# chao1224/GeoSSL

Measured on AMD Instinct MI355X. Metric: molecules/s/GPU SchNet+DDM fwd+bwd (QM9-sized, bs=1024); % HBM roofline, higher is better.
Workload: dtype f32

## Files before the change

geossl_amd/csrc/aggregate_reg.h:

```cpp
#pragma once
#include "common.h"

namespace geossl {

typedef float f32x2 __attribute__((ext_vector_type(2)));

template <int NMAX, int RING_ = 0>
__device__ __forceinline__ void aggregate_reg_body(const float* __restrict__ x, const float* __restrict__ Wf,
                                                   const uint8_t* __restrict__ pair_flag, int a0, int n, int base,
                                                   int lane, int f, int F, int swap, float* __restrict__ out) {
#pragma clang fp contract(off)
  typedef f32x2 V;
#ifndef AGG_RING_SMALL
#define AGG_RING_SMALL 16
#endif
  constexpr int RING = RING_ > 0 ? RING_ : (NMAX > 26 ? 24 : (NMAX > 20 ? 20 : (NMAX > 18 ? 12 : AGG_RING_SMALL)));
  constexpr int NPOS = NMAX * (NMAX - 1) / 2;
  const float* __restrict__ wbase = Wf + (size_t)base * F;
  const bool has_cols = f >= 0;
  f = has_cols ? f : 0;
  if (n < 2) {
    if (n == 1 && has_cols) *reinterpret_cast<V*>(out + (size_t)a0 * F + f) = V(0.0f);
    return;
  }
  V xr[NMAX], acc[NMAX], ring[RING];
#pragma unroll
  for (int i = 0; i < NMAX; ++i) {
    xr[i] = *reinterpret_cast<const V*>(x + (size_t)(a0 + min(i, n - 1)) * F + f);
    acc[i] = V(0.0f);
  }
  const int nu = __builtin_amdgcn_readfirstlane(n);
  int rs_req = 0;
  auto load_row = [&](int a, int b) {
    asm volatile("" : "+s"(rs_req));
    const int slot = b < nu ? rs_req + (b - a - 1) : 0;
    const float* rowp = wbase + (size_t)slot * F;
    return __builtin_nontemporal_load(reinterpret_cast<const V*>(rowp + f));
  };
  auto next_pos = [&](int& a, int& b) {
    if (++b == NMAX) {
      rs_req += nu - a - 1;
      ++a;
      b = a + 1;
    }
  };
  unsigned flr[NMAX - 1];
#pragma unroll
  for (int a = 0; a < NMAX - 1; ++a) {
    const bool mine = lane > a && lane < n;
    flr[a] = pair_flag[base + (mine ? a * n - a * (a + 1) / 2 + lane - a - 1 : 0)];
  }
  int q = 0, ap = 0, bp = 1;
#pragma unroll
  for (int k = 0; k < RING && k < NPOS; ++k) {
    ring[k] = load_row(ap, bp);
    next_pos(ap, bp);
  }
#pragma unroll
  for (int a = 0; a < NMAX - 1; ++a) {
    const bool mine = lane > a && lane < n;
    unsigned fl = flr[a];
    asm volatile("" : "+v"(fl));
    fl = mine ? fl : 0u;
    if (swap) fl = ((fl & 1u) << 1) | ((fl >> 1) & 1u);
    const unsigned long long m0 = __builtin_amdgcn_ballot_w64((fl & 1u) != 0u);
    const unsigned long long m1 = __builtin_amdgcn_ballot_w64((fl & 2u) != 0u);
    V acc_a = acc[a];
    const V xa = xr[a];
#pragma unroll
    for (int b = a + 1; b < NMAX; ++b, ++q) {
      const V w = ring[q % RING];
      if (q + RING < NPOS) {
        ring[q % RING] = load_row(ap, bp);
        next_pos(ap, bp);
      }
      const V t0 = xr[b] * w;
      const V s0 = acc_a + t0;
      acc_a = ((m0 >> b) & 1ull) ? s0 : acc_a;
      const V t1 = xa * w;
      const V s1 = acc[b] + t1;
      acc[b] = ((m1 >> b) & 1ull) ? s1 : acc[b];
      asm volatile("" : "+v"(acc_a.x), "+v"(acc_a.y), "+v"(acc[b].x), "+v"(acc[b].y) : : "memory");
      __builtin_amdgcn_sched_barrier(0);
    }
    acc[a] = acc_a;
  }
#pragma unroll
  for (int i = 0; i < NMAX; ++i)
    if (i < n && has_cols) *reinterpret_cast<V*>(out + (size_t)(a0 + i) * F + f) = acc[i];
}

template <int NW = 4>
__device__ __forceinline__ void aggregate_block_body(const float* __restrict__ x, const float* __restrict__ Wf,
                                                     const uint8_t* __restrict__ pair_flag, int a0, int n, int base,
                                                     int swap, float* __restrict__ out, uint8_t* smem) {
#pragma clang fp contract(off)
  typedef f32x2 V;
  constexpr int F = 128, NP = 32;
  float* xs = reinterpret_cast<float*>(smem);
  uint8_t* fls = smem + 33 * F * sizeof(float);
  const int tid = threadIdx.x, lane = tid & 63;
  const int wave = __builtin_amdgcn_readfirstlane(tid >> 6);
  const int nu = __builtin_amdgcn_readfirstlane(n), np = nu * (nu - 1) / 2;
  for (int i = tid; i < nu * (F / 4); i += 64 * NW) {
    const int row = i >> 5, q = i & 31;
    *reinterpret_cast<f32x4*>(xs + row * F + 4 * q) = *reinterpret_cast<const f32x4*>(x + (size_t)(a0 + row) * F + 4 * q);
  }
  for (int p = tid; p < np; p += 64 * NW) {
    unsigned fl = pair_flag[base + p];
    if (swap) fl = ((fl & 1u) << 1) | ((fl >> 1) & 1u);
    fls[p] = (uint8_t)fl;
  }
  __syncthreads();
  if (nu < 2) {
    if (nu == 1 && wave == 0) *reinterpret_cast<V*>(out + (size_t)a0 * F + 2 * lane) = V(0.0f);
    return;
  }
  const float* __restrict__ wcol = Wf + (size_t)base * F + 2 * lane;
  const float* xl = xs + 2 * lane;
  int slot_l = 0, b_l = 0;
  unsigned long long mask = 0ull;
  auto describe = [&](int a) {
// ... 216 lines not shown
```

geossl_amd/csrc/chain.hip:

```cpp
#include "common.h"
#include "geossl_hip.h"
#include "split.h"
#ifdef LOOP_TIMING
__device__ long long loop_dbg[2 * 1024];
__device__ int loop_dbg_n;
#define LOOP_MARK(tag)                                                                                     \
  do {                                                                                                     \
    if (blockIdx.x == 5 && threadIdx.x == 64) {                                                            \
      const int k_ = loop_dbg_n;                                                                           \
      if (k_ < 1024) {                                                                                     \
        loop_dbg[2 * k_] = (tag);                                                                          \
        loop_dbg[2 * k_ + 1] = (long long)__builtin_amdgcn_s_memrealtime();                                \
        loop_dbg_n = k_ + 1;                                                                               \
      }                                                                                                    \
    }                                                                                                      \
  } while (0)
#else
#define LOOP_MARK(tag) do {} while (0)
#endif
#include "aggregate_reg.h"

#include <cstdlib>

using namespace geossl;
// ... 462 lines not shown
                  const u32x4* src = xs + (size_t)((ks + 1) * 3) * 64;
                  xn.h = src[0]; xn.m = src[64]; xn.l = src[128];
                }
                __builtin_amdgcn_sched_barrier(0);
                mma6(acc, af[ks], xa);
                __builtin_amdgcn_sched_barrier(0);
                if (ks + 1 < KS) xa = xn;
              }
            }
            epilogue(st, m, acc, tp, rs, v);
            if (s + 1 < NS) {
              const float lo[8] = {v[0], v[1], v[2], v[3], v[4], v[5], v[6], v[7]};
              const float hi[8] = {v[8], v[9], v[10], v[11], v[12], v[13], v[14], v[15]};
              const Frag3 f0 = split8(lo), f1 = split8(hi);
              u32x4* xd = xchg + (size_t)(s & 1) * CHUNK + (size_t)(2 * m * 3) * 64 + lane;
              xd[0] = f0.h; xd[64] = f0.m; xd[128] = f0.l;
              xd[192] = f1.h; xd[256] = f1.m; xd[320] = f1.l;
            }
          }
          __syncthreads();
          if (active && mbc == 0) store_v(st, m, ro, live, v);
          if (cc + NSLOT < total) issue(cc + NSLOT);
        }
      }
    }
  }
}

__device__ __forceinline__ float silu_f(float x) { return x / (1.0f + expf(-x)); }
__device__ __forceinline__ float dsilu_f(float x) {
  const float sg = 1.0f / (1.0f + expf(-x));
  return sg * (1.0f + x * (1.0f - sg));
}
template <int NS, int RB, int WPS, bool SILU, typename ChainT>
__device__ __forceinline__ void chain_cu_body(const ChainT& ch, const float* __restrict__ X, int ldx, int R,
                                              int row0, int row_end, int nloc) {
  constexpr int KS = 8, F = 128;
  constexpr int RBF = KS * 2 * 64;
#ifndef CHAIN_CU_NEB2
#define CHAIN_CU_NEB2 1
#endif
  constexpr int NEB = WPS == 1 ? 2 : CHAIN_CU_NEB2;
  extern __shared__ __attribute__((aligned(16))) uint8_t smem_raw[];
  u32x4* xbuf = reinterpret_cast<u32x4*>(smem_raw);
  float* bias_s = reinterpret_cast<float*>(xbuf + (size_t)RB * RBF);
  float* rmax = bias_s + NS * F;
  const int tid = threadIdx.x, lane = tid & 63, j = lane & 31, kh = lane >> 5;
  const int m = __builtin_amdgcn_readfirstlane(tid >> 6);
  const uint32_t voff = (uint32_t)lane * 16u;
  Frag2 af[KS];
  int eW = 0;
  float krow[RB];
  auto request_weights = [&](const auto& st) __attribute__((always_inline)) {
    const char* img = reinterpret_cast<const char*>(st.image) + (size_t)(m * KS) * 2 * 1024;
#pragma unroll
    for (int ks = 0; ks < KS; ++ks) {
      const char* bk = img + ks * 2 * 1024;
      asm volatile("" : "+s"(bk));
      af[ks].h = *reinterpret_cast<const u32x4*>(bk + voff);
      af[ks].l = *reinterpret_cast<const u32x4*>(bk + 1024 + voff);
    }
    eW = reinterpret_cast<const int*>(st.image)[4 * KS * 2 * 64 * 4 + m];
  };
  auto publish_max = [&](int i, float mx) __attribute__((always_inline)) {
    mx = fmaxf(mx, __shfl_xor(mx, 32, 64));
    if (kh == 0) rmax[(i * 4 + m) * 32 + j] = mx;
  };
  auto row_scale = [&](int i) __attribute__((always_inline)) {
    const float* r = rmax + (i * 4) * 32 + j;
    const float mx = fmaxf(fmaxf(r[0], r[32]), fmaxf(r[64], r[96]));
    const int e = mag_exponent(mx);
    krow[i] = __builtin_amdgcn_ldexpf(1.0f, e - 14);
    return __builtin_amdgcn_ldexpf(1.0f, 14 - e);
  };
  request_weights(ch.st[0]);
  for (int i = tid; i < NS * F; i += 256) {
    const int s = i / F;
    bias_s[i] = ch.st[s].bias != nullptr ? ch.st[s].bias[i - s * F] : 0.0f;
  }
  auto load_input = [&](const float* __restrict__ Xp, int ldxp) __attribute__((always_inline)) {
    f32x4 raw[RB][4];
    const char* xb = reinterpret_cast<const char*>(Xp) + 128 * m;
#pragma unroll
    for (int i = 0; i < RB; ++i) {
      const uint32_t rowc = (uint32_t)min(row0 + 32 * min(i, nloc - 1) + j, row_end - 1);
      const uint32_t xo = rowc * (uint32_t)ldxp * 4u + 16u * kh;
#pragma unroll
      for (int q = 0; q < 4; ++q) raw[i][q] = *reinterpret_cast<const f32x4*>(xb + 32 * q + xo);
    }
#pragma unroll
    for (int i = 0; i < RB; ++i) {
      if (i < nloc) {
        float mx = 0.0f;
#pragma unroll
        for (int q = 0; q < 4; ++q)
          mx = fmaxf(fmaxf(mx, fmaxf(fabsf(raw[i][q].x), fabsf(raw[i][q].y))), fmaxf(fabsf(raw[i][q].z), fabsf(raw[i][q].w)));
        publish_max(i, mx);
      }
    }
    lds_barrier();
#pragma unroll
    for (int i = 0; i < RB; ++i) {
      if (i < nloc) {
        const float sr = row_scale(i);
        const float lo[8] = {raw[i][0].x, raw[i][0].y, raw[i][0].z, raw[i][0].w,
                             raw[i][1].x, raw[i][1].y, raw[i][1].z, raw[i][1].w};
        const float hi[8] = {raw[i][2].x, raw[i][2].y, raw[i][2].z, raw[i][2].w,
                             raw[i][3].x, raw[i][3].y, raw[i][3].z, raw[i][3].w};
        const Frag2 f0 = split8h_scaled(lo, sr), f1 = split8h_scaled(hi, sr);
        u32x4* xd = xbuf + (size_t)i * RBF + (size_t)(2 * m * 2) * 64 + lane;
        xd[0] = f0.h; xd[64] = f0.l;
        xd[128] = f1.h; xd[192] = f1.l;
      }
    }
  };
  load_input(X, ldx);
  lds_barrier();
  LOOP_MARK(100);
  float vout[RB][16];
#pragma unroll
  for (int s = 0; s < NS; ++s) {
    const auto st = ch.st[s];
    const int eWs = eW;
    f32x4 tp[NEB][4], rs[NEB][4];
    const uint32_t nbytes = (uint32_t)R * (uint32_t)st.ld * 4u;
    const __amdgpu_buffer_rsrc_t rs_t = __builtin_amdgcn_make_buffer_rsrc(const_cast<float*>(st.tprev), 0, st.tprev != nullptr ? nbytes : 0u, 0x00020000);
    const __amdgpu_buffer_rsrc_t rs_r = __builtin_amdgcn_make_buffer_rsrc(const_cast<float*>(st.res), 0, st.res != nullptr ? nbytes : 0u, 0x00020000);
    const __amdgpu_buffer_rsrc_t rs_o = __builtin_amdgcn_make_buffer_rsrc(st.out, 0, st.out != nullptr ? nbytes : 0u, 0x00020000);
    const __amdgpu_buffer_rsrc_t rs_a = __builtin_amdgcn_make_buffer_rsrc(st.out_act, 0, (SILU && st.out_act != nullptr) ? nbytes : 0u, 0x00020000);
    const bool act_silu = SILU && (st.flags & GEOSSL_EPI_SILU) != 0;
    auto row_off = [&](int i) __attribute__((always_inline)) {
      const int row = row0 + 32 * i + j;
      return row < row_end ? (uint32_t)row * (uint32_t)st.ld * 4u + 128u * m + 16u * kh : 0xFFFFFF00u;
    };
    auto request_epi = [&](int i, f32x4 (&t)[4], f32x4 (&r)[4]) __attribute__((always_inline)) {
      const uint32_t ro = row_off(i);
#pragma unroll
      for (int q = 0; q < 4; ++q) t[q] = __builtin_bit_cast(f32x4, __builtin_amdgcn_raw_buffer_load_b128(rs_t, ro + 32 * q, 0, 0));
#pragma unroll
      for (int q = 0; q < 4; ++q) r[q] = __builtin_bit_cast(f32x4, __builtin_amdgcn_raw_buffer_load_b128(rs_r, ro + 32 * q, 0, 0));
    };
    auto store_rb = [&](int i) __attribute__((always_inline)) {
      const uint32_t ro = row_off(i);
#pragma unroll
      for (int q = 0; q < 4; ++q)
        __builtin_amdgcn_raw_buffer_store_b128(
            __builtin_bit_cast(u32x4, f32x4{vout[i][4 * q], vout[i][4 * q + 1], vout[i][4 * q + 2], vout[i][4 * q + 3]}), rs_o,
            ro + 32 * q, 0, 0);
      if constexpr (SILU) {
// ... 72 lines not shown
#pragma unroll
          for (int q = 0; q < 4; ++q) {
            vout[i][4 * q] *= dssp_from_out(t[q].x);
            vout[i][4 * q + 1] *= dssp_from_out(t[q].y);
            vout[i][4 * q + 2] *= dssp_from_out(t[q].z);
            vout[i][4 * q + 3] *= dssp_from_out(t[q].w);
          }
        }
        if (st.res != nullptr) {
#pragma unroll
          for (int q = 0; q < 4; ++q) {
            vout[i][4 * q] += r[q].x;
            vout[i][4 * q + 1] += r[q].y;
            vout[i][4 * q + 2] += r[q].z;
            vout[i][4 * q + 3] += r[q].w;
          }
        }
        if (s + 1 < NS) {
          float mx = 0.0f;
#pragma unroll
          for (int e = 0; e < 16; ++e) mx = fmaxf(mx, fabsf(vout[i][e]));
          publish_max(i, mx);
        }
        if (i > 0) store_rb(i - 1);
        if (i + 1 == nloc) store_rb(i);
      }
    }
    LOOP_MARK(110 + s);
    if (s + 1 < NS) {
      request_weights(ch.st[s + 1]);
      if (ch.st[s + 1].flags & GEOSSL_CHAIN_SAME_INPUT) continue;
      lds_barrier();
      if (ch.st[s + 1].flags & GEOSSL_CHAIN_NEW_INPUT) {
        load_input(ch.st[s + 1].xin, ch.st[s + 1].ldxin);
        lds_barrier();
        continue;
      }
#pragma unroll
      for (int i = 0; i < RB; ++i) {
        if (i < nloc) {
          const float sr = row_scale(i);
          float lo[8], hi[8];
#pragma unroll
          for (int e = 0; e < 8; ++e) {
            lo[e] = vout[i][e];
            hi[e] = vout[i][8 + e];
          }
          if constexpr (SILU) {
            if (st.flags & GEOSSL_EPI_SILU) {
#pragma unroll
              for (int e = 0; e < 8; ++e) {
                lo[e] = silu_f(lo[e]);
                hi[e] = silu_f(hi[e]);
              }
            }
          }
          const Frag2 f0 = split8h_scaled(lo, sr), f1 = split8h_scaled(hi, sr);
          u32x4* xd = xbuf + (size_t)i * RBF + (size_t)(2 * m * 2) * 64 + lane;
          xd[0] = f0.h; xd[64] = f0.l;
          xd[128] = f1.h; xd[192] = f1.l;
        }
      }
      lds_barrier();
    }
  }
}

template <int NS, int RB, int WPS, bool SILU>
__global__ __launch_bounds__(256, WPS) void k_row_chain_cu(GeosslChain ch, const float* __restrict__ X, int ldx, int R,
                                                           const int32_t* __restrict__ dyn_R) {
  R = dyn_count(R, dyn_R);
  const int nrb = (R + 31) / 32;
  const int nblk = (int)gridDim.x, base = nrb / nblk, extra = nrb - base * nblk, b = (int)blockIdx.x;
  const int rb0 = b * base + min(b, extra);
  const int nloc = base + (b < extra ? 1 : 0);
  if (nloc == 0) return;
  chain_cu_body<NS, RB, WPS, SILU>(ch, X, ldx, R, 32 * rb0, R, nloc);
}

struct LoopStage {
  const uint32_t* image;
  const float* bias;
  const float* res;
  const float* tprev;
  float* out;
  int flags, pad;
  static constexpr int ld = 128, ldxin = 0;
  static constexpr const float* xin = nullptr;
  static constexpr float* out_act = nullptr;
};
struct LoopOp {
  const float* X;
  const float* Wf;
  float* out;
  int kind, nstage, swap, pad;
  LoopStage st[3];
};
constexpr int LOOP_MAX_OPS = 14;
struct LoopArgs {
  LoopOp op[LOOP_MAX_OPS];
  const int4* plan;
  const int32_t* mol_ptr;
  const int32_t* pair_ptr;
  const uint8_t* pair_flag;
  int nops, R, stagger, pad;
  int nmol, mols_per_block;
};

template <int NMAX, int NW = 4>
__global__ __launch_bounds__(64 * NW, NW == 4 ? 2 : 1) void k_layer_loop(LoopArgs a) {
  constexpr int F = 128;
  int4 pl;
  if constexpr (NMAX > 0) {
    pl = a.plan[blockIdx.x];
  } else {
    pl.z = (int)blockIdx.x * a.mols_per_block;
    pl.w = min(pl.z + a.mols_per_block, a.nmol);
    if (pl.z >= pl.w) return;
    pl.x = a.mol_ptr[pl.z];
    pl.y = a.mol_ptr[pl.w];
    if (pl.x >= pl.y) return;
  }
  const int nloc = (pl.y - pl.x + 31) / 32;
  const int wave = __builtin_amdgcn_readfirstlane((int)threadIdx.x >> 6), lane = threadIdx.x & 63;
  if ((int)blockIdx.x >= ((int)gridDim.x + 1) / 2)
    for (int i = 0; i < a.stagger; ++i) __builtin_amdgcn_s_sleep(127);
  LOOP_MARK(1);
  for (int o = 0; o < a.nops; ++o) {
    const LoopOp& op = a.op[o];
    LOOP_MARK(10 + op.kind);
    if (op.kind == 0) {
      if (NW > 4 && wave >= 4) {
        for (int i = 0; i < 2 * op.nstage; ++i) __builtin_amdgcn_s_barrier();
      } else if (op.nstage == 1) chain_cu_body<1, 3, 2, false>(op, op.X, F, a.R, pl.x, pl.y, nloc);
      else if (op.nstage == 2) chain_cu_body<2, 3, 2, false>(op, op.X, F, a.R, pl.x, pl.y, nloc);
      else chain_cu_body<3, 3, 2, false>(op, op.X, F, a.R, pl.x, pl.y, nloc);
    } else {
      if constexpr (NMAX > 0 && NW == 4) {
        for (int mm = pl.z + wave; mm < pl.w; mm += 4) {
          const int a0 = a.mol_ptr[mm], n = a.mol_ptr[mm + 1] - a0, base = a.pair_ptr[mm];
          aggregate_reg_body<NMAX>(op.X, op.Wf, a.pair_flag, a0, n, base, lane, 2 * lane, F, op.swap, op.out);
        }
      } else {
        extern __shared__ __attribute__((aligned(16))) uint8_t loop_smem[];
        for (int mm = pl.z; mm < pl.w; ++mm) {
          const int a0 = a.mol_ptr[mm], n = a.mol_ptr[mm + 1] - a0, base = a.pair_ptr[mm];
          if (mm > pl.z) __syncthreads();
          aggregate_block_body<NW>(op.X, op.Wf, a.pair_flag, a0, n, base, op.swap, op.out, loop_smem);
        }
      }
    }
    LOOP_MARK(20);
    asm volatile("s_waitcnt vmcnt(0)" ::: "memory");
    LOOP_MARK(21);
    __syncthreads();
  }
  LOOP_MARK(2);
}

template <int KS>
int launch_chain(const GeosslChain& ch, const float* X, int ldx, int64_t R, hipStream_t stream,
                 const int32_t* dyn_R = nullptr) {
  constexpr int NMB = KS / 2, CHUNK_BYTES = KS * 3 * 1024;
  if (dyn_R != nullptr && KS != 8) return (int)hipErrorInvalidValue;
  const int nrb = (int)((R + 31) / 32), ngroups = (nrb + 3) / 4;
  const int nslot = chain_slots(ch.nstage * NMB);
  static const bool four_waves = getenv("GEOSSL_CHAIN4") != nullptr;
  static const bool eight_waves = getenv("GEOSSL_CHAIN8") != nullptr;
  const bool cu_form = KS == 8;
  const bool offsets32 = cu_form || !four_waves;
  bool same_input = false, silu = false;
  for (int s2 = 0; s2 < ch.nstage; ++s2) silu |= (ch.st[s2].flags & (GEOSSL_EPI_SILU | GEOSSL_EPI_MUL_DSILU)) != 0;
  if (ch.nstage > 3) silu = true;
  if (silu && !cu_form) return (int)hipErrorInvalidValue;
  for (int s2 = 0; s2 < ch.nstage; ++s2) {
    if (offsets32 && ((int64_t)R * ch.st[s2].ld * 4 >= (int64_t)0xFFFFFF00u || (int64_t)R * ldx * 4 >= (int64_t)0xFFFFFF00u ||
                      (int64_t)R * ch.st[s2].ldxin * 4 >= (int64_t)0xFFFFFF00u)) {
// ... 178 lines not shown
    } else if (src.kind == 1) {
      if (src.Wf == nullptr || src.out == nullptr) return (int)hipErrorInvalidValue;
      for (int s2 = 0; s2 < 3; ++s2) d.st[s2] = LoopStage{nullptr, nullptr, nullptr, nullptr, nullptr, 0, 0};
    } else {
      return (int)hipErrorInvalidValue;
    }
  }
  return 0;
}

static bool loop_wide(int64_t nblocks, bool one_molecule_per_block) {
  static int cus = 0;
  if (cus == 0) {
    int dev = 0, n = 0;
    cus = (hipGetDevice(&dev) == hipSuccess &&
           hipDeviceGetAttribute(&n, hipDeviceAttributeMultiprocessorCount, dev) == hipSuccess && n > 0) ? n : -1;
  }
  return one_molecule_per_block && cus > 0 && nblocks <= cus && getenv("GEOSSL_LOOP_NO_WIDE") == nullptr;
}

extern "C" int geossl_schnet_layer_loop(const GeosslLoopOp* ops, int nops, const int32_t* plan, int nblocks,
                                        const int32_t* mol_ptr, const int32_t* pair_ptr, const uint8_t* pair_flag,
                                        int max_n, int uniform, int64_t N, int F, int stagger, hipStream_t stream) {
  if (nops <= 0 || nblocks <= 0) return 0;
  if (ops == nullptr || plan == nullptr || nops > LOOP_MAX_OPS || F != 128 || !uniform || max_n > 20 || N <= 0)
    return (int)hipErrorInvalidValue;
  if (N * (int64_t)F * 4 >= (int64_t)0xFFFFFF00u) return (int)hipErrorInvalidValue;
  LoopArgs a;
  const int rc = fill_loop_ops(ops, nops, F, a);
  if (rc != 0) return rc;
  a.plan = reinterpret_cast<const int4*>(plan);
  a.mol_ptr = mol_ptr; a.pair_ptr = pair_ptr; a.pair_flag = pair_flag;
  a.nops = nops; a.R = (int)N; a.stagger = stagger; a.pad = 0; a.nmol = 0; a.mols_per_block = 0;
  const size_t lds = (size_t)3 * 8 * 2 * 1024 + (size_t)3 * 128 * sizeof(float) + (size_t)3 * 128 * sizeof(float);
  if (max_n <= 18) {
    allow_big_lds(&k_layer_loop<18>);
    hipLaunchKernelGGL((k_layer_loop<18>), dim3(nblocks), dim3(256), lds, stream, a);
  } else {
    allow_big_lds(&k_layer_loop<20>);
    hipLaunchKernelGGL((k_layer_loop<20>), dim3(nblocks), dim3(256), lds, stream, a);
  }
  GEOSSL_CHECK_LAUNCH();
  return 0;
}

extern "C" int geossl_schnet_layer_loop_ragged(const GeosslLoopOp* ops, int nops, const int32_t* mol_ptr,
                                               const int32_t* pair_ptr, const uint8_t* pair_flag, int64_t B,
                                               int mols_per_block, int64_t N, int F, hipStream_t stream) {
  if (nops <= 0 || B <= 0) return 0;
  if (ops == nullptr || mol_ptr == nullptr || pair_ptr == nullptr || nops > LOOP_MAX_OPS || F != 128 || N <= 0 ||
      mols_per_block < 1 || mols_per_block > 2)
    return (int)hipErrorInvalidValue;
  if (N * (int64_t)F * 4 >= (int64_t)0xFFFFFF00u) return (int)hipErrorInvalidValue;
  const int64_t nblocks = (B + mols_per_block - 1) / mols_per_block;
  if (nblocks > 1024) return (int)hipErrorInvalidValue;
  LoopArgs a;
  const int rc = fill_loop_ops(ops, nops, F, a);
  if (rc != 0) return rc;
  a.plan = nullptr;
  a.mol_ptr = mol_ptr; a.pair_ptr = pair_ptr; a.pair_flag = pair_flag;
  a.nops = nops; a.R = (int)N; a.stagger = 0; a.pad = 0; a.nmol = (int)B; a.mols_per_block = mols_per_block;
  const size_t lds = (size_t)3 * 8 * 2 * 1024 + (size_t)3 * 128 * sizeof(float) + (size_t)3 * 128 * sizeof(float);
  if (loop_wide(nblocks, mols_per_block == 1)) {
    allow_big_lds(&k_layer_loop<0, 8>);
    hipLaunchKernelGGL((k_layer_loop<0, 8>), dim3((unsigned)nblocks), dim3(512), lds, stream, a);
  } else {
// ... 7 lines not shown
```

geossl_amd/csrc/common.h:

```cpp
#pragma once
#include <hip/hip_runtime.h>
#include <stdint.h>

#include <mutex>

typedef float f32x16 __attribute__((ext_vector_type(16)));
typedef float f32x4 __attribute__((ext_vector_type(4)));

#define GEOSSL_MAX_LAYERS 12
#define GEOSSL_PI_F 3.14159265358979323846f

#define GEOSSL_CHECK_LAUNCH()                  \
  do {                                         \
    hipError_t e__ = hipGetLastError();        \
    if (e__ != hipSuccess) return (int)e__;    \
  } while (0)

namespace geossl {

inline void allow_big_lds_ptr(const void* kernel) {
  struct Seen { const void* fn; int dev; };
  static Seen seen[512];
  static int nseen = 0;
  static std::mutex mu;
// ... 75 lines not shown
    }
    asm volatile("s_waitcnt lgkmcnt(0)" ::: "memory");
#pragma unroll
    for (int u = 0; u < 2; ++u) {
      const int row16 = 8 * u + rr;
      const float4 v = *reinterpret_cast<const float4*>(stage + row16 * 32 + 4 * c4);
      consume(16 * half + row16, 4 * c4, v);
    }
    asm volatile("s_waitcnt lgkmcnt(0)" ::: "memory");
  }
}

__device__ __forceinline__ float pin(float v) {
  asm volatile("" : "+v"(v));
  return v;
}
__device__ __forceinline__ float4 pin(float4 v) {
  asm volatile("" : "+v"(v.x), "+v"(v.y), "+v"(v.z), "+v"(v.w));
  return v;
}

__device__ __forceinline__ float kahan_sum_strided(const float* __restrict__ p, int b0, int b1, int stride) {
#pragma clang fp reassociate(off) contract(off)
  float s = 0.0f, c = 0.0f;
#pragma unroll 4
  for (int b = b0; b < b1; ++b) {
    const float y = p[(size_t)b * stride] - c;
    const float t = s + y;
    c = (t - s) - y;
    s = t;
  }
  return s;
}

__device__ __forceinline__ int dyn_count(int cap, const int32_t* __restrict__ dyn) {
  return dyn != nullptr ? min(cap, *dyn) : cap;
}

__device__ __forceinline__ float wave_sum(float v) {
#pragma unroll
  for (int o = 32; o > 0; o >>= 1) v += __shfl_xor(v, o, 64);
  return v;
}

__device__ __forceinline__ float sigmoidf_(float v) { return 1.0f / (1.0f + expf(-v)); }
__device__ __forceinline__ float siluf_(float v) { return v / (1.0f + expf(-v)); }
__device__ __forceinline__ double softplus_d(double z) { return fmax(z, 0.0) + log1p(exp(-fabs(z))); }
__device__ __forceinline__ double sigmoid_d(double z) { return 1.0 / (1.0 + exp(-z)); }

enum Readout { kAdd = 0, kMean = 1, kExternal = 2 };

__device__ __forceinline__ float readout_col(const float* __restrict__ h, int F, int j, int a0, int a1, bool mean) {
  float acc = 0.0f;
  for (int a = a0; a < a1; ++a) acc += h[(size_t)a * F + j];
  return mean ? acc / fmaxf((float)(a1 - a0), 1.0f) : acc;
}
__device__ __forceinline__ float readout_grad(float g, int a0, int a1, bool mean) {
  return mean ? g / fmaxf((float)(a1 - a0), 1.0f) : g;
}
__device__ __forceinline__ void scatter_readout_col(float* __restrict__ dh, int F, int j, int a0, int a1, float g,
                                                    bool mean, bool accumulate = false) {
  const float gv = readout_grad(g, a0, a1, mean);
  for (int a = a0; a < a1; ++a) {
    const size_t o = (size_t)a * F + j;
    dh[o] = accumulate ? dh[o] + gv : gv;
  }
// ... 4 lines not shown
```

geossl_amd/csrc/ddm.hip:

```cpp
#include "common.h"
#include "geossl_hip.h"
#include "tn.h"
#include "wgrad.h"

using namespace geossl;

namespace {

inline int grid1d(int64_t n, int block, int cap = 2048) {
  int64_t g = (n + block - 1) / block;
  return (int)(g < 1 ? 1 : (g > cap ? cap : g));
}

__global__ __launch_bounds__(256) void k_sum_partial(const float* __restrict__ x, int64_t n, float* __restrict__ partial) {
  __shared__ float red[256];
  const int64_t per = (n + gridDim.x - 1) / gridDim.x;
  const int64_t lo = blockIdx.x * per, hi = min(n, lo + per);
  float s = 0.0f;
  for (int64_t i = lo + threadIdx.x; i < hi; i += 256) s += x[i];
  red[threadIdx.x] = s;
  __syncthreads();
  for (int o = 128; o > 0; o >>= 1) {
    if (threadIdx.x < o) red[threadIdx.x] += red[threadIdx.x + o];
    __syncthreads();
// ... 195 lines not shown
  const int a = grp * 4 + (threadIdx.x >> 6), lane = threadIdx.x & 63;
  if (a >= N) return;
  const int64_t p0 = inc_ptr[a], p1 = inc_ptr[a + 1];
  float acc[4] = {0.0f, 0.0f, 0.0f, 0.0f};
  if (accumulate) {
#pragma unroll
    for (int v = 0; v < 4; ++v)
      if (lane + 64 * v < F) acc[v] = dh[(size_t)a * F + lane + 64 * v];
  }
  for (int64_t pb = p0; pb < p1; pb += 64) {
    const int cnt = (int)min((int64_t)64, p1 - pb);
    const int mine = lane < cnt ? inc_idx[pb + lane] : 0;
    for (int q0 = 0; q0 < cnt; q0 += 8) {
      float val[8][4];
#pragma unroll
      for (int u = 0; u < 8; ++u) {
        const int s = __shfl(mine, min(q0 + u, cnt - 1), 64);
#pragma unroll
        for (int v = 0; v < 4; ++v)
          if (lane + 64 * v < F) val[u][v] = dfeat[(size_t)s * F + lane + 64 * v];
      }
#pragma unroll
      for (int u = 0; u < 8; ++u)
        if (q0 + u < cnt) {
#pragma unroll
          for (int v = 0; v < 4; ++v)
            if (lane + 64 * v < F) acc[v] += val[u][v];
        }
    }
  }
#pragma unroll
  for (int v = 0; v < 4; ++v)
    if (lane + 64 * v < F) dh[(size_t)a * F + lane + 64 * v] = acc[v];
}

__global__ void k_adam(float* __restrict__ p, const float* __restrict__ g, float* __restrict__ m,
                       float* __restrict__ v, int64_t n, float step_size, float w1, float beta2, float w2, float eps,
                       float wd, float bc2_sqrt, float grad_scale) {
  for (int64_t i = (int64_t)blockIdx.x * blockDim.x + threadIdx.x; i < n; i += (int64_t)gridDim.x * blockDim.x) {
    float gi = mul_rn(g[i], grad_scale);
    const float pi = p[i];
    if (wd != 0.0f) gi = fmaf(wd, pi, gi);
    const float m0 = m[i];
    const float mi = fmaf(w1, add_rn(gi, -m0), m0);
    const float vi = fmaf(w2, mul_rn(gi, gi), mul_rn(v[i], beta2));
    m[i] = mi;
    v[i] = vi;
    const float denom = add_rn(sqrtf(vi) / bc2_sqrt, eps);
    p[i] = fmaf(-step_size, mi / denom, pi);
  }
}

}

namespace geossl {
int launch_ncsn_small_reduce(const float* partial, int nblk, int F, const GeosslNcsnGrads& g, int accumulate,
                             hipStream_t stream);
}

extern "C" int64_t geossl_loss_reduce_workspace_floats(int64_t S) { return GEOSSL_LOSS_BLOCKS; }

extern "C" int geossl_loss_reduce(const float* loss_e, int64_t S, const int64_t* stats_divisor, float out_scale,
                                  float* loss, float* workspace, int accumulate, hipStream_t stream) {
  hipLaunchKernelGGL(k_sum_partial, dim3(GEOSSL_LOSS_BLOCKS), dim3(256), 0, stream, loss_e, S, workspace);
  GEOSSL_CHECK_LAUNCH();
  hipLaunchKernelGGL(k_loss_final, dim3(1), dim3(64), 0, stream, workspace, GEOSSL_LOSS_BLOCKS, stats_divisor, out_scale,
// ... 44 lines not shown
  int rc;
  o.dW[0] = grads->o2_w;
  o.db[0] = grads->o2_b;
  NcsnW2Ops l2{grow, w->o3_w, saved->a2, saved->a1, F, H};
  if (F == 128) rc = launch_wgrad_split<2, 4>(l2, 1, S, H, F, o, F, 1, workspace, accumulate, stream);
  else if (F == 64) rc = launch_wgrad_split<1, 2>(l2, 1, S, H, F, o, F, 1, workspace, accumulate, stream);
  else rc = launch_wgrad_split<1, 1>(l2, 1, S, H, F, o, F, 1, workspace, accumulate, stream);
  if (rc) return rc;
  o.dW[0] = grads->o1_w;
  o.db[0] = grads->o1_b;
  o.dd[0] = grads->o1_w + F;
  NcsnW1Ops l1{dz1, h, sei0, sei1, saved->emb, F};
  if (F == 128) rc = launch_wgrad_split<4, 4>(l1, 1, S, F, F, o, F + 1, F + 1, workspace, accumulate, stream);
  else if (F == 64) rc = launch_wgrad_split<2, 2>(l1, 1, S, F, F, o, F + 1, F + 1, workspace, accumulate, stream);
  else rc = launch_wgrad_split<1, 1>(l1, 1, S, F, F, o, F + 1, F + 1, workspace, accumulate, stream);
  if (rc) return rc;
  int chunk, nblk;
  small_plan(S, &chunk, &nblk);
  hipLaunchKernelGGL(k_ncsn_small_partial, dim3(nblk), dim3(128), 0, stream, *w, *saved, grow, demb, (int)S, F, chunk,
                     workspace);
  GEOSSL_CHECK_LAUNCH();
  return launch_ncsn_small_reduce(workspace, nblk, F, *grads, accumulate, stream);
}

namespace geossl {
int launch_ncsn_small_reduce(const float* partial, int nblk, int F, const GeosslNcsnGrads& g, int accumulate,
                             hipStream_t stream) {
  hipLaunchKernelGGL(k_ncsn_small_reduce, dim3(F / 2 + 3 * F + 2), dim3(64), 0, stream, partial, nblk, F, g, accumulate);
  GEOSSL_CHECK_LAUNCH();
  return 0;
}
}

extern "C" int geossl_incidence_gather(const float* dfeat, const int64_t* inc_ptr, const int32_t* inc_idx, int64_t N,
                                       int F, float* dh, int accumulate, hipStream_t stream) {
  if (N <= 0) return 0;
  const unsigned groups = (unsigned)((N + 3) / 4);
  hipLaunchKernelGGL(k_incidence_gather, dim3((groups + 7) / 8 * 8), dim3(256), 0, stream, dfeat, inc_ptr, inc_idx,
                     (int)N, F, dh, accumulate, (const float*)nullptr, (float*)nullptr, (const int32_t*)nullptr);
  GEOSSL_CHECK_LAUNCH();
  return 0;
}

namespace geossl {
int launch_incidence_gather2(const float* dfeat0, const float* dfeat1, const int64_t* inc_ptr, const int32_t* inc_idx,
                             int64_t N, int F, float* dh0, float* dh1, hipStream_t stream, const int32_t* dyn_view) {
  if (N <= 0) return 0;
  const unsigned groups = (unsigned)((N + 3) / 4);
  hipLaunchKernelGGL(k_incidence_gather, dim3((groups + 7) / 8 * 8, 2), dim3(256), 0, stream, dfeat0, inc_ptr, inc_idx,
                     (int)N, F, dh0, 0, dfeat1, dh1, dyn_view);
  GEOSSL_CHECK_LAUNCH();
  return 0;
}
}

extern "C" int geossl_adam_step(float* param, const float* grad, float* exp_avg, float* exp_avg_sq, int64_t n, double lr,
                                double beta1, double beta2, double eps, double weight_decay, int64_t step_count,
                                float grad_scale, hipStream_t stream) {
  if (n <= 0) return 0;
  const double bc1 = 1.0 - pow(beta1, (double)step_count);
  const double bc2 = 1.0 - pow(beta2, (double)step_count);
  hipLaunchKernelGGL(k_adam, dim3(grid1d(n, 256)), dim3(256), 0, stream, param, grad, exp_avg, exp_avg_sq, n,
                     (float)(lr / bc1), (float)(1.0 - beta1), (float)beta2, (float)(1.0 - beta2), (float)eps,
                     (float)weight_decay, (float)sqrt(bc2), grad_scale);
  GEOSSL_CHECK_LAUNCH();
  return 0;
}
```

geossl_amd/csrc/schnet.hip:

```cpp
#include "common.h"
#include "aggregate_reg.h"
#include "geossl_hip.h"
#include "tn.h"

#include <cstdlib>

using namespace geossl;

namespace {

inline int grid1d(int64_t n, int block, int cap = 2048) {
  int64_t g = (n + block - 1) / block;
  return (int)(g < 1 ? 1 : (g > cap ? cap : g));
}

__global__ void k_rbf(const float* __restrict__ d, int64_t E, const float* __restrict__ offset, int G, float coeff,
                      float* __restrict__ out) {
  for (int64_t i = (int64_t)blockIdx.x * blockDim.x + threadIdx.x; i < E * G; i += (int64_t)gridDim.x * blockDim.x) {
    const int64_t e = i / G;
    const int g = (int)(i - e * G);
    const float diff = d[e] - offset[g];
    out[i] = expf(coeff * (diff * diff));
  }
}
// ... 262 lines not shown
__global__ __launch_bounds__(256) void k_embedding_fwd4(const int64_t* __restrict__ z, int64_t zs,
                                                        const float* __restrict__ table, int C, int N,
                                                        float* __restrict__ out, int32_t* __restrict__ status,
                                                        const int32_t* __restrict__ dyn_N) {
  N = dyn_count(N, dyn_N);
  const uint32_t total = (uint32_t)N << SH4;
  for (uint32_t i = blockIdx.x * 256u + threadIdx.x; i < total; i += gridDim.x * 256u) {
    const uint32_t a = i >> SH4, f4 = i & ((1u << SH4) - 1u);
    const int64_t c = z[(int64_t)a * zs];
    f32x4 v = {0.0f, 0.0f, 0.0f, 0.0f};
    if (c < 0 || c >= C) {
      if (status != nullptr) *status = 1;
    } else {
      v = reinterpret_cast<const f32x4*>(table)[((uint32_t)c << SH4) + f4];
    }
    reinterpret_cast<f32x4*>(out)[i] = v;
  }
}

#define GEOSSL_EMB_CHUNKS 512
template <int NG>
__global__ void k_embedding_bwd_partial(const int64_t* __restrict__ z, int64_t zs, const float* __restrict__ dh,
                                        int64_t N, int F, int C, float* __restrict__ partial, int2* __restrict__ band,
                                        const int32_t* __restrict__ dyn_N) {
  extern __shared__ __attribute__((aligned(16))) float smem[];
  N = dyn_count((int)N, dyn_N);
  const int TF = blockDim.x / NG;
  const int chunk = blockIdx.x, grp = threadIdx.x / TF, f = threadIdx.x - grp * TF;
  const int64_t per = (N + (int64_t)gridDim.x - 1) / (int64_t)gridDim.x;
  const int64_t lo = chunk * per, hi = min((int64_t)N, lo + per);
  float* tab = smem + (size_t)grp * C * F;
  int2* gband = reinterpret_cast<int2*>(smem + (size_t)NG * C * F);
  int cmin = C, cmax = -1;
  if (f < F) {
    for (int c = 0; c < C; ++c) tab[c * F + f] = 0.0f;
    constexpr int U = 16;
    for (int64_t a0 = lo + grp; a0 < hi; a0 += (int64_t)U * NG) {
      float v[U];
      int cls[U];
#pragma unroll
      for (int u = 0; u < U; ++u) {
        const int64_t a = min(a0 + (int64_t)u * NG, hi - 1);
        v[u] = dh[a * F + f];
        const int64_t c64 = z[a * zs];
        cls[u] = (c64 >= 0 && c64 < C) ? (int)c64 : -1;
      }
#pragma unroll
      for (int u = 0; u < U; ++u)
        if (a0 + (int64_t)u * NG < hi && cls[u] >= 0 && cls[u] < C) {
          tab[cls[u] * F + f] += v[u];
          cmin = min(cmin, cls[u]);
          cmax = max(cmax, cls[u]);
        }
    }
    if (f == 0) gband[grp] = make_int2(cmin, cmax);
  }
  if (NG > 1) {
    __syncthreads();
    if (grp != 0) return;
    for (int g = 0; g < NG; ++g) {
      cmin = min(cmin, gband[g].x);
      cmax = max(cmax, gband[g].y);
    }
  }
  if (f >= F) return;
  for (int c = cmin; c <= cmax; ++c) {
    float sum = smem[c * F + f];
    for (int g = 1; g < NG; ++g) sum += smem[((size_t)g * C + c) * F + f];
    partial[((size_t)chunk * C + c) * F + f] = sum;
  }
  if (f == 0) band[chunk] = make_int2(cmin, cmax);
}
__global__ __launch_bounds__(256) void k_embedding_bwd_reduce(const float* __restrict__ partial,
                                                              const int2* __restrict__ band, int nchunks, int C, int F,
                                                              float* __restrict__ dtable, int accumulate) {
  constexpr int PERMAX = GEOSSL_EMB_CHUNKS / 4;
  static_assert(PERMAX == 128, "two chunks per lane");
  const int PER = nchunks / 4;
  __shared__ float red[4][64];
  __shared__ int hits[4][PERMAX];
  const int c = blockIdx.y, lane = threadIdx.x & 63, slice = threadIdx.x >> 6;
  const int f = blockIdx.x * 64 + lane;
  int n = 0;
#pragma unroll
  for (int h = 0; h < 2; ++h) {
    const int b = slice * PER + 64 * h + lane;
    const int2 r = 64 * h + lane < PER ? band[b] : make_int2(1, 0);
    const bool hit = c >= r.x && c <= r.y;
    const unsigned long long m = __ballot(hit);
    if (hit) hits[slice][n + __popcll(m & ((1ull << lane) - 1ull))] = b;
    n += __popcll(m);
  }
  __builtin_amdgcn_wave_barrier();
  float s = 0.0f;
  if (f < F) {
#pragma clang fp reassociate(off) contract(off)
    float k = 0.0f;
    const float* p = partial + (size_t)c * F + f;
#pragma unroll 4
    for (int i = 0; i < n; ++i) {
      const float y = p[(size_t)hits[slice][i] * C * F] - k;
      const float t = s + y;
      k = (t - s) - y;
      s = t;
    }
  }
  red[slice][lane] = s;
  __syncthreads();
  if (slice == 0 && f < F) {
    float v = accumulate ? dtable[(size_t)c * F + f] : 0.0f;
    v += red[0][lane];
    v += red[1][lane];
    v += red[2][lane];
    v += red[3][lane];
    dtable[(size_t)c * F + f] = v;
  }
}
__global__ void k_segment_reduce_fwd(const float* __restrict__ h, const int32_t* __restrict__ mol_ptr, int B, int F,
                                     int mean, float* __restrict__ out) {
  const int m = blockIdx.x;
  if (m >= B) return;
  const int a0 = mol_ptr[m], a1 = mol_ptr[m + 1];
  for (int f = threadIdx.x; f < F; f += blockDim.x) out[(size_t)m * F + f] = readout_col(h, F, f, a0, a1, mean != 0);
}
__global__ void k_segment_reduce_bwd(const float* __restrict__ dout, const int32_t* __restrict__ mol_ptr, int B, int F,
                                     int mean, float* __restrict__ dh, int accumulate) {
  const int m = blockIdx.x;
  if (m >= B) return;
  const int a0 = mol_ptr[m], a1 = mol_ptr[m + 1];
  for (int f = threadIdx.x; f < F; f += blockDim.x)
    scatter_readout_col(dh, F, f, a0, a1, dout[(size_t)m * F + f], mean != 0, accumulate != 0);
}

__global__ __launch_bounds__(256) void k_row_normalize_fwd(const float* __restrict__ h, int64_t N, int F, float eps,
                                                           float* __restrict__ y, float* __restrict__ norm) {
  const int lane = threadIdx.x & 63;
  const int64_t row = (int64_t)blockIdx.x * 4 + (threadIdx.x >> 6);
  if (row >= N) return;
// ... 234 lines not shown
```

Baseline: 414,100.

## Hand off intermediate rows between chain and aggregate ops through LDS

When consecutive ops in the fused layer loop are a dense chain and an aggregation, and one writes the buffer the other reads, the producer now also writes its rows into a swizzled LDS row buffer. The consumer then reads its inputs from LDS instead of re-reading them from global memory. The aim is to cut the global round-trip between ops. The global store is still performed, and the LDS region reuses the chain's xbuf, which relies on barrier ordering and on each block's rows fitting in the three row blocks.

```diff
diff --git a/geossl_amd/csrc/aggregate_reg.h b/geossl_amd/csrc/aggregate_reg.h
--- a/geossl_amd/csrc/aggregate_reg.h
+++ b/geossl_amd/csrc/aggregate_reg.h
@@ -5,12 +5,21 @@
 
 typedef float f32x2 __attribute__((ext_vector_type(2)));
 
-template <int NMAX, int RING_ = 0>
+__device__ __forceinline__ uint32_t hand_row_off(int row, int chunk) {
+  return (uint32_t)row * 512u + ((uint32_t)(chunk ^ (row & 15)) << 4);
+}
+constexpr int HAND_IN = 1;
+constexpr int HAND_OUT = 2;
+
+template <int NMAX, int RING_ = 0, bool HAND = false>
 __device__ __forceinline__ void aggregate_reg_body(const float* __restrict__ x, const float* __restrict__ Wf,
                                                    const uint8_t* __restrict__ pair_flag, int a0, int n, int base,
-                                                   int lane, int f, int F, int swap, float* __restrict__ out) {
+                                                   int lane, int f, int F, int swap, float* __restrict__ out,
+                                                   uint8_t* rowbuf = nullptr, int lrow0 = 0) {
 #pragma clang fp contract(off)
   typedef f32x2 V;
+  const int hand = HAND ? swap >> 1 : 0;
+  if constexpr (HAND) swap &= 1;
 #ifndef AGG_RING_SMALL
 #define AGG_RING_SMALL 16
 #endif
@@ -19,15 +28,28 @@
   const float* __restrict__ wbase = Wf + (size_t)base * F;
   const bool has_cols = f >= 0;
   f = has_cols ? f : 0;
+  auto hand_ptr = [&](int r) { return reinterpret_cast<V*>(rowbuf + hand_row_off(r, lane >> 1) + 8 * (lane & 1)); };
   if (n < 2) {
-    if (n == 1 && has_cols) *reinterpret_cast<V*>(out + (size_t)a0 * F + f) = V(0.0f);
+    if (n == 1 && has_cols) {
+      *reinterpret_cast<V*>(out + (size_t)a0 * F + f) = V(0.0f);
+      if constexpr (HAND)
+        if (hand & HAND_OUT) *hand_ptr(lrow0) = V(0.0f);
+    }
     return;
   }
   V xr[NMAX], acc[NMAX], ring[RING];
-#pragma unroll
-  for (int i = 0; i < NMAX; ++i) {
-    xr[i] = *reinterpret_cast<const V*>(x + (size_t)(a0 + min(i, n - 1)) * F + f);
-    acc[i] = V(0.0f);
+  if (HAND && (hand & HAND_IN)) {
+#pragma unroll
+    for (int i = 0; i < NMAX; ++i) {
+      xr[i] = *hand_ptr(lrow0 + min(i, n - 1));
+      acc[i] = V(0.0f);
+    }
+  } else {
+#pragma unroll
+    for (int i = 0; i < NMAX; ++i) {
+      xr[i] = *reinterpret_cast<const V*>(x + (size_t)(a0 + min(i, n - 1)) * F + f);
+      acc[i] = V(0.0f);
+    }
   }
   const int nu = __builtin_amdgcn_readfirstlane(n);
   int rs_req = 0;
@@ -88,6 +110,13 @@
 #pragma unroll
   for (int i = 0; i < NMAX; ++i)
     if (i < n && has_cols) *reinterpret_cast<V*>(out + (size_t)(a0 + i) * F + f) = acc[i];
+  if constexpr (HAND) {
+    if (hand & HAND_OUT) {
+#pragma unroll
+      for (int i = 0; i < NMAX; ++i)
+        if (i < n) *hand_ptr(lrow0 + i) = acc[i];
+    }
+  }
 }
 
 template <int NW = 4>
diff --git a/geossl_amd/csrc/chain.hip b/geossl_amd/csrc/chain.hip
--- a/geossl_amd/csrc/chain.hip
+++ b/geossl_amd/csrc/chain.hip
@@ -518,9 +518,10 @@
   const float sg = 1.0f / (1.0f + expf(-x));
   return sg * (1.0f + x * (1.0f - sg));
 }
-template <int NS, int RB, int WPS, bool SILU, typename ChainT>
+template <int NS, int RB, int WPS, bool SILU, bool HAND = false, typename ChainT>
 __device__ __forceinline__ void chain_cu_body(const ChainT& ch, const float* __restrict__ X, int ldx, int R,
-                                              int row0, int row_end, int nloc) {
+                                              int row0, int row_end, int nloc, int hand = 0) {
+  static_assert(!HAND || RB == 3, "the row buffer is the three row blocks of xbuf");
   constexpr int KS = 8, F = 128;
   constexpr int RBF = KS * 2 * 64;
 #ifndef CHAIN_CU_NEB2
@@ -564,15 +565,25 @@
     const int s = i / F;
     bias_s[i] = ch.st[s].bias != nullptr ? ch.st[s].bias[i - s * F] : 0.0f;
   }
-  auto load_input = [&](const float* __restrict__ Xp, int ldxp) __attribute__((always_inline)) {
+  auto load_input = [&](const float* __restrict__ Xp, int ldxp, bool from_rowbuf) __attribute__((always_inline)) {
     f32x4 raw[RB][4];
     const char* xb = reinterpret_cast<const char*>(Xp) + 128 * m;
-#pragma unroll
-    for (int i = 0; i < RB; ++i) {
-      const uint32_t rowc = (uint32_t)min(row0 + 32 * min(i, nloc - 1) + j, row_end - 1);
-      const uint32_t xo = rowc * (uint32_t)ldxp * 4u + 16u * kh;
-#pragma unroll
-      for (int q = 0; q < 4; ++q) raw[i][q] = *reinterpret_cast<const f32x4*>(xb + 32 * q + xo);
+    if (HAND && from_rowbuf) {
+#pragma unroll
+      for (int i = 0; i < RB; ++i) {
+        const int rowl = min(32 * min(i, nloc - 1) + j, row_end - 1 - row0);
+#pragma unroll
+        for (int q = 0; q < 4; ++q)
+          raw[i][q] = *reinterpret_cast<const f32x4*>(smem_raw + hand_row_off(rowl, 8 * m + 2 * q + kh));
+      }
+    } else {
+#pragma unroll
+      for (int i = 0; i < RB; ++i) {
+        const uint32_t rowc = (uint32_t)min(row0 + 32 * min(i, nloc - 1) + j, row_end - 1);
+        const uint32_t xo = rowc * (uint32_t)ldxp * 4u + 16u * kh;
+#pragma unroll
+        for (int q = 0; q < 4; ++q) raw[i][q] = *reinterpret_cast<const f32x4*>(xb + 32 * q + xo);
+      }
     }
 #pragma unroll
     for (int i = 0; i < RB; ++i) {
@@ -600,7 +611,7 @@
       }
     }
   };
-  load_input(X, ldx);
+  load_input(X, ldx, (hand & HAND_IN) != 0);
   lds_barrier();
   LOOP_MARK(100);
   float vout[RB][16];
@@ -739,7 +750,7 @@
       if (ch.st[s + 1].flags & GEOSSL_CHAIN_SAME_INPUT) continue;
       lds_barrier();
       if (ch.st[s + 1].flags & GEOSSL_CHAIN_NEW_INPUT) {
-        load_input(ch.st[s + 1].xin, ch.st[s + 1].ldxin);
+        load_input(ch.st[s + 1].xin, ch.st[s + 1].ldxin, false);
         lds_barrier();
         continue;
       }
@@ -769,6 +780,20 @@
         }
       }
       lds_barrier();
+    }
+    if constexpr (HAND) {
+      if (s + 1 == NS && (hand & HAND_OUT)) {
+        lds_barrier();
+#pragma unroll
+        for (int i = 0; i < RB; ++i) {
+          if (i < nloc) {
+#pragma unroll
+            for (int q = 0; q < 4; ++q)
+              *reinterpret_cast<f32x4*>(smem_raw + hand_row_off(32 * i + j, 8 * m + 2 * q + kh)) =
+                  f32x4{vout[i][4 * q], vout[i][4 * q + 1], vout[i][4 * q + 2], vout[i][4 * q + 3]};
+          }
+        }
+      }
     }
   }
 }
@@ -830,26 +855,31 @@
   }
   const int nloc = (pl.y - pl.x + 31) / 32;
   const int wave = __builtin_amdgcn_readfirstlane((int)threadIdx.x >> 6), lane = threadIdx.x & 63;
+  constexpr bool HAND = NMAX > 0 && NW == 4;
+  extern __shared__ __attribute__((aligned(16))) uint8_t loop_smem[];
   if ((int)blockIdx.x >= ((int)gridDim.x + 1) / 2)
     for (int i = 0; i < a.stagger; ++i) __builtin_amdgcn_s_sleep(127);
   LOOP_MARK(1);
   for (int o = 0; o < a.nops; ++o) {
     const LoopOp& op = a.op[o];
     LOOP_MARK(10 + op.kind);
+    const int hand = HAND ? op.pad : 0;
+    int row0 = pl.x, row_end = pl.y, nlo = nloc;
+    if constexpr (HAND) asm volatile("" : "+s"(row0), "+s"(row_end), "+s"(nlo));
     if (op.kind == 0) {
       if (NW > 4 && wave >= 4) {
         for (int i = 0; i < 2 * op.nstage; ++i) __builtin_amdgcn_s_barrier();
-      } else if (op.nstage == 1) chain_cu_body<1, 3, 2, false>(op, op.X, F, a.R, pl.x, pl.y, nloc);
-      else if (op.nstage == 2) chain_cu_body<2, 3, 2, false>(op, op.X, F, a.R, pl.x, pl.y, nloc);
-      else chain_cu_body<3, 3, 2, false>(op, op.X, F, a.R, pl.x, pl.y, nloc);
+      } else if (op.nstage == 1) chain_cu_body<1, 3, 2, false, HAND>(op, op.X, F, a.R, row0, row_end, nlo, hand);
+      else if (op.nstage == 2) chain_cu_body<2, 3, 2, false, HAND>(op, op.X, F, a.R, row0, row_end, nlo, hand);
+      else chain_cu_body<3, 3, 2, false, HAND>(op, op.X, F, a.R, row0, row_end, nlo, hand);
     } else {
       if constexpr (NMAX > 0 && NW == 4) {
         for (int mm = pl.z + wave; mm < pl.w; mm += 4) {
           const int a0 = a.mol_ptr[mm], n = a.mol_ptr[mm + 1] - a0, base = a.pair_ptr[mm];
-          aggregate_reg_body<NMAX>(op.X, op.Wf, a.pair_flag, a0, n, base, lane, 2 * lane, F, op.swap, op.out);
+          aggregate_reg_body<NMAX, 0, HAND>(op.X, op.Wf, a.pair_flag, a0, n, base, lane, 2 * lane, F,
+                                            HAND ? op.swap | (hand << 1) : op.swap, op.out, loop_smem, a0 - row0);
         }
       } else {
-        extern __shared__ __attribute__((aligned(16))) uint8_t loop_smem[];
         for (int mm = pl.z; mm < pl.w; ++mm) {
           const int a0 = a.mol_ptr[mm], n = a.mol_ptr[mm + 1] - a0, base = a.pair_ptr[mm];
           if (mm > pl.z) __syncthreads();
@@ -1094,6 +1124,18 @@
   a.plan = reinterpret_cast<const int4*>(plan);
   a.mol_ptr = mol_ptr; a.pair_ptr = pair_ptr; a.pair_flag = pair_flag;
   a.nops = nops; a.R = (int)N; a.stagger = stagger; a.pad = 0; a.nmol = 0; a.mols_per_block = 0;
+  const char* hand_env = getenv("GEOSSL_LOOP_HANDOFF");
+  if (hand_env == nullptr || atoi(hand_env) != 0) {
+    for (int o = 0; o + 1 < nops; ++o) {
+      LoopOp& p = a.op[o];
+      LoopOp& q = a.op[o + 1];
+      const float* written = p.kind == 0 ? p.st[p.nstage - 1].out : p.out;
+      if (p.kind != q.kind && written != nullptr && written == q.X) {
+        p.pad |= HAND_OUT;
+        q.pad |= HAND_IN;
+      }
+    }
+  }
   const size_t lds = (size_t)3 * 8 * 2 * 1024 + (size_t)3 * 128 * sizeof(float) + (size_t)3 * 128 * sizeof(float);
   if (max_n <= 18) {
     allow_big_lds(&k_layer_loop<18>);
```

After: 399,500. 0.965x the previous value.

## Add F=128 float4 incidence gather and batch loads in embedding backward

Applied to the files above, without the earlier changes.

Adds a specialised incidence-gather kernel for F=128 in which each half-wave handles one atom with float4 loads, broadcasts neighbour indices through readlane, and issues up to 20 independent row loads before accumulating. The embedding backward partial kernel now loads 32 rows per iteration and fetches the class ids once per wave, broadcasting them with readlane instead of each lane reloading them. The reduce kernel's Kahan loop is batched so its loads are issued ahead of the serial compensated adds. The aim is more memory-level parallelism and fewer scalar loads on these bandwidth-bound gathers, at the cost of higher register pressure and an extra code path gated on alignment.

```diff
diff --git a/geossl_amd/csrc/common.h b/geossl_amd/csrc/common.h
--- a/geossl_amd/csrc/common.h
+++ b/geossl_amd/csrc/common.h
@@ -131,6 +131,39 @@
   }
   return s;
 }
+__device__ __forceinline__ void kahan_add(float& s, float& c, float v) {
+#pragma clang fp reassociate(off) contract(off)
+  const float y = v - c;
+  const float t = s + y;
+  c = (t - s) - y;
+  s = t;
+}
+template <int U, class AtFn>
+__device__ __forceinline__ void kahan_batch(float& s, float& c, int i, AtFn at) {
+  float v[U];
+#pragma unroll
+  for (int u = 0; u < U; ++u) v[u] = *at(i + u);
+#pragma unroll
+  for (int u = 0; u < U; ++u) kahan_add(s, c, v[u]);
+}
+template <int U, class AtFn>
+__device__ __forceinline__ void kahan_tail(float& s, float& c, int& i, int n, AtFn at) {
+  if constexpr (U >= 1) {
+    if (i + U <= n) {
+      kahan_batch<U>(s, c, i, at);
+      i += U;
+    }
+    kahan_tail<U / 2>(s, c, i, n, at);
+  }
+}
+template <int UMAX, class AtFn>
+__device__ __forceinline__ float kahan_sum_batched(int n, AtFn at) {
+  float s = 0.0f, c = 0.0f;
+  int i = 0;
+  for (; i + UMAX <= n; i += UMAX) kahan_batch<UMAX>(s, c, i, at);
+  kahan_tail<UMAX / 2>(s, c, i, n, at);
+  return s;
+}
 
 __device__ __forceinline__ int dyn_count(int cap, const int32_t* __restrict__ dyn) {
   return dyn != nullptr ? min(cap, *dyn) : cap;
diff --git a/geossl_amd/csrc/ddm.hip b/geossl_amd/csrc/ddm.hip
--- a/geossl_amd/csrc/ddm.hip
+++ b/geossl_amd/csrc/ddm.hip
@@ -251,6 +251,51 @@
 #pragma unroll
   for (int v = 0; v < 4; ++v)
     if (lane + 64 * v < F) dh[(size_t)a * F + lane + 64 * v] = acc[v];
+}
+
+#define GATHER_U 20
+__global__ __launch_bounds__(256) void k_incidence_gather128(const float* __restrict__ dfeat0,
+                                                             const int64_t* __restrict__ inc_ptr,
+                                                             const int32_t* __restrict__ inc_idx, int N,
+                                                             float* __restrict__ dh0, int accumulate,
+                                                             const float* __restrict__ dfeat1, float* __restrict__ dh1,
+                                                             const int32_t* __restrict__ dyn_view) {
+  constexpr int F = 128;
+  const float* __restrict__ dfeat = blockIdx.y == 0 ? dfeat0 : dfeat1;
+  float* __restrict__ dh = blockIdx.y == 0 ? dh0 : dh1;
+  N = dyn_count(N, dyn_view);
+  if (dyn_view != nullptr && blockIdx.y == 1) dh += (size_t)N * F;
+  const int per = ((int)gridDim.x + 7) / 8;
+  const int grp = ((int)blockIdx.x % 8) * per + (int)blockIdx.x / 8;
+  const int a = grp * 8 + (threadIdx.x >> 5), hl = threadIdx.x & 31;
+  if (a >= N) return;
+  const int64_t p0 = inc_ptr[a], p1 = inc_ptr[a + 1];
+  float4* __restrict__ drow = reinterpret_cast<float4*>(dh + (size_t)a * F) + hl;
+  float4 acc = {0.0f, 0.0f, 0.0f, 0.0f};
+  if (accumulate) acc = *drow;
+  for (int64_t pb = p0; pb < p1; pb += 32) {
+    const int cnt = (int)min((int64_t)32, p1 - pb);
+    const int mine = hl < cnt ? inc_idx[pb + hl] : 0;
+    for (int q0 = 0; q0 < cnt; q0 += GATHER_U) {
+      float4 val[GATHER_U];
+#pragma unroll
+      for (int u = 0; u < GATHER_U; ++u) {
+        const int k = (q0 + u) & 31;
+        const int slo = __builtin_amdgcn_readlane(mine, k), shi = __builtin_amdgcn_readlane(mine, 32 + k);
+        const int s = (threadIdx.x & 32) ? shi : slo;
+        if (q0 + u < cnt) val[u] = reinterpret_cast<const float4*>(dfeat + (size_t)s * F)[hl];
+      }
+#pragma unroll
+      for (int u = 0; u < GATHER_U; ++u)
+        if (q0 + u < cnt) {
+          acc.x += val[u].x;
+          acc.y += val[u].y;
+          acc.z += val[u].z;
+          acc.w += val[u].w;
+        }
+    }
+  }
+  *drow = acc;
 }
 
 __global__ void k_adam(float* __restrict__ p, const float* __restrict__ g, float* __restrict__ m,
@@ -361,25 +406,34 @@
 }
 }
 
+static int launch_gather(const float* dfeat0, const float* dfeat1, const int64_t* inc_ptr, const int32_t* inc_idx,
+                         int64_t N, int F, float* dh0, float* dh1, int accumulate, int heads, const int32_t* dyn_view,
+                         hipStream_t stream) {
+  const uintptr_t bits = (uintptr_t)dfeat0 | (uintptr_t)dfeat1 | (uintptr_t)dh0 | (uintptr_t)dh1;
+  if (F == 128 && (bits & 15) == 0) {
+    const unsigned groups = (unsigned)((N + 7) / 8);
+    hipLaunchKernelGGL(k_incidence_gather128, dim3((groups + 7) / 8 * 8, heads), dim3(256), 0, stream, dfeat0, inc_ptr,
+                       inc_idx, (int)N, dh0, accumulate, dfeat1, dh1, dyn_view);
+  } else {
+    const unsigned groups = (unsigned)((N + 3) / 4);
+    hipLaunchKernelGGL(k_incidence_gather, dim3((groups + 7) / 8 * 8, heads), dim3(256), 0, stream, dfeat0, inc_ptr,
+                       inc_idx, (int)N, F, dh0, accumulate, dfeat1, dh1, dyn_view);
+  }
+  GEOSSL_CHECK_LAUNCH();
+  return 0;
+}
+
 extern "C" int geossl_incidence_gather(const float* dfeat, const int64_t* inc_ptr, const int32_t* inc_idx, int64_t N,
                                        int F, float* dh, int accumulate, hipStream_t stream) {
   if (N <= 0) return 0;
-  const unsigned groups = (unsigned)((N + 3) / 4);
-  hipLaunchKernelGGL(k_incidence_gather, dim3((groups + 7) / 8 * 8), dim3(256), 0, stream, dfeat, inc_ptr, inc_idx,
-                     (int)N, F, dh, accumulate, (const float*)nullptr, (float*)nullptr, (const int32_t*)nullptr);
-  GEOSSL_CHECK_LAUNCH();
-  return 0;
+  return launch_gather(dfeat, nullptr, inc_ptr, inc_idx, N, F, dh, nullptr, accumulate, 1, nullptr, stream);
 }
 
 namespace geossl {
 int launch_incidence_gather2(const float* dfeat0, const float* dfeat1, const int64_t* inc_ptr, const int32_t* inc_idx,
                              int64_t N, int F, float* dh0, float* dh1, hipStream_t stream, const int32_t* dyn_view) {
   if (N <= 0) return 0;
-  const unsigned groups = (unsigned)((N + 3) / 4);
-  hipLaunchKernelGGL(k_incidence_gather, dim3((groups + 7) / 8 * 8, 2), dim3(256), 0, stream, dfeat0, inc_ptr, inc_idx,
-                     (int)N, F, dh0, 0, dfeat1, dh1, dyn_view);
-  GEOSSL_CHECK_LAUNCH();
-  return 0;
+  return launch_gather(dfeat0, dfeat1, inc_ptr, inc_idx, N, F, dh0, dh1, 0, 2, dyn_view, stream);
 }
 }
 
diff --git a/geossl_amd/csrc/schnet.hip b/geossl_amd/csrc/schnet.hip
--- a/geossl_amd/csrc/schnet.hip
+++ b/geossl_amd/csrc/schnet.hip
@@ -318,29 +318,28 @@
   float* tab = smem + (size_t)grp * C * F;
   int2* gband = reinterpret_cast<int2*>(smem + (size_t)NG * C * F);
   int cmin = C, cmax = -1;
-  if (f < F) {
+  const bool on = f < F;
+  const int fc = on ? f : 0, wl = threadIdx.x & 63;
+  if (on)
     for (int c = 0; c < C; ++c) tab[c * F + f] = 0.0f;
-    constexpr int U = 16;
-    for (int64_t a0 = lo + grp; a0 < hi; a0 += (int64_t)U * NG) {
-      float v[U];
-      int cls[U];
-#pragma unroll
-      for (int u = 0; u < U; ++u) {
-        const int64_t a = min(a0 + (int64_t)u * NG, hi - 1);
-        v[u] = dh[a * F + f];
-        const int64_t c64 = z[a * zs];
-        cls[u] = (c64 >= 0 && c64 < C) ? (int)c64 : -1;
+  constexpr int U = 32;
+  for (int64_t a0 = lo + grp; a0 < hi; a0 += (int64_t)U * NG) {
+    float v[U];
+    const int64_t c64 = z[min(a0 + (int64_t)(wl & (U - 1)) * NG, hi - 1) * zs];
+    const int mycls = (c64 >= 0 && c64 < C) ? (int)c64 : -1;
+#pragma unroll
+    for (int u = 0; u < U; ++u) v[u] = dh[min(a0 + (int64_t)u * NG, hi - 1) * F + fc];
+#pragma unroll
+    for (int u = 0; u < U; ++u) {
+      const int cls = __builtin_amdgcn_readlane(mycls, u);
+      if (a0 + (int64_t)u * NG < hi && cls >= 0 && on) {
+        tab[cls * F + f] += v[u];
+        cmin = min(cmin, cls);
+        cmax = max(cmax, cls);
       }
-#pragma unroll
-      for (int u = 0; u < U; ++u)
-        if (a0 + (int64_t)u * NG < hi && cls[u] >= 0 && cls[u] < C) {
-          tab[cls[u] * F + f] += v[u];
-          cmin = min(cmin, cls[u]);
-          cmax = max(cmax, cls[u]);
-        }
-    }
-    if (f == 0) gband[grp] = make_int2(cmin, cmax);
-  }
+    }
+  }
+  if (f == 0) gband[grp] = make_int2(cmin, cmax);
   if (NG > 1) {
     __syncthreads();
     if (grp != 0) return;
@@ -380,16 +379,9 @@
   __builtin_amdgcn_wave_barrier();
   float s = 0.0f;
   if (f < F) {
-#pragma clang fp reassociate(off) contract(off)
-    float k = 0.0f;
     const float* p = partial + (size_t)c * F + f;
-#pragma unroll 4
-    for (int i = 0; i < n; ++i) {
-      const float y = p[(size_t)hits[slice][i] * C * F] - k;
-      const float t = s + y;
-      k = (t - s) - y;
-      s = t;
-    }
+    const int* hl = hits[slice];
+    s = kahan_sum_batched<32>(n, [&](int i) { return p + (size_t)hl[i] * C * F; });
   }
   red[slice][lane] = s;
   __syncthreads();
```

After: 425,500 before, 429,800 after (median of 6 runs). +1.0%, better.
